# Drexubery/ViewCrafter

Measured on NVIDIA H100. Metric: DDIM denoise-steps/sec @ 576x1024x25f, higher is better.
Workload: dtype f16 (fp32 accumulate; fp32 norms/softmax/update)

## Files before the change

### viewcrafter_b200/csrc/attention.cu

```cuda
#include <cstdlib>

#include "common.cuh"
#include "kernels.h"
#include "wgmma.cuh"

namespace vc {

struct AttnParams {
  CUtensorMap tmap_q, tmap_k, tmap_v;
  __half* out;
  int ldo;
  int Nq, Nk;
  int kv_shared;
  float scale_log2;
  int accumulate;
};

static constexpr int ATT_BM = 128, ATT_D = 64;
static constexpr int ATT_THREADS = 288;
static constexpr int ATT_Q_BYTES = ATT_BM * ATT_D * 2;

template <int BNK>
struct AttnCfg {
  static constexpr int KV_BYTES = BNK * ATT_D * 2;
  static constexpr int SMEM = ATT_Q_BYTES + 4 * KV_BYTES + 1024 + 256;
  static constexpr int MIN_CTAS = BNK == 64 ? 2 : 1;
};

__device__ __forceinline__ float ex2f(float x) {
  float y;
  asm("ex2.approx.ftz.f32 %0, %1;" : "=f"(y) : "f"(x));
  return y;
}

template <int BNK>
__global__ void __launch_bounds__(ATT_THREADS, AttnCfg<BNK>::MIN_CTAS) flash_attn_d64_kernel(const __grid_constant__ AttnParams p) {
  using Cfg = AttnCfg<BNK>;
  extern __shared__ uint8_t smem_raw[];
  uint8_t* smem = reinterpret_cast<uint8_t*>((reinterpret_cast<uintptr_t>(smem_raw) + 1023) & ~uintptr_t(1023));
  uint8_t* sQ = smem;
  uint8_t* sKV = smem + ATT_Q_BYTES;
  uint64_t* bars = reinterpret_cast<uint64_t*>(smem + ATT_Q_BYTES + 4 * Cfg::KV_BYTES);
  uint64_t* q_full = bars + 0;
  uint64_t* kv_full = bars + 1;
  uint64_t* kv_empty = bars + 3;

  const int warp = threadIdx.x >> 5, lane = threadIdx.x & 31;
  const int q0 = blockIdx.x * ATT_BM, head = blockIdx.y, b = blockIdx.z;
  const int bk = p.kv_shared ? 0 : b;
  const int ntiles = (p.Nk + BNK - 1) / BNK;

  if (threadIdx.x == 0) {
    tma_prefetch_desc(&p.tmap_q);
    tma_prefetch_desc(&p.tmap_k);
    tma_prefetch_desc(&p.tmap_v);
    mbar_init(q_full, 1);
    mbar_init(&kv_full[0], 1); mbar_init(&kv_full[1], 1);
    mbar_init(&kv_empty[0], 8); mbar_init(&kv_empty[1], 8);
    fence_barrier_init();
  }
  __syncthreads();

  if (warp == 8) {
    if (elect_one()) {
      mbar_expect_tx(q_full, ATT_Q_BYTES);
      tma_load_4d(sQ, &p.tmap_q, q_full, 0, head, q0, b);
    }
    __syncwarp();
    for (int j = 0; j < ntiles; ++j) {
      const int s = j & 1;
      uint8_t* sk = sKV + s * 2 * Cfg::KV_BYTES;
      if (j >= 2) mbar_wait(&kv_empty[s], ((j >> 1) - 1) & 1);
      if (elect_one()) {
        mbar_expect_tx(&kv_full[s], 2 * Cfg::KV_BYTES);
        tma_load_4d(sk, &p.tmap_k, &kv_full[s], 0, head, j * BNK, bk);
        tma_load_4d(sk + Cfg::KV_BYTES, &p.tmap_v, &kv_full[s], 0, head, j * BNK, bk);
      }
      __syncwarp();
    }
    return;
  }

  const int cw = warp >> 2, wl = warp & 3;
  const uint32_t aQ = smem_u32(sQ) + cw * (64 * ATT_D * 2);
  const float sl2 = p.scale_log2;
  float o[32];
#pragma unroll
  for (int i = 0; i < 32; ++i) o[i] = 0.f;
  float m[2] = {-INFINITY, -INFINITY}, l[2] = {0.f, 0.f};
  mbar_wait(q_full, 0);
  for (int j = 0; j < ntiles; ++j) {
    const int s = j & 1;
    const uint32_t aK = smem_u32(sKV + s * 2 * Cfg::KV_BYTES);
    const uint32_t aV = aK + Cfg::KV_BYTES;
    mbar_wait(&kv_full[s], (j >> 1) & 1);
    float sc[BNK / 2];
    wgmma_fence();
#pragma unroll
    for (int k = 0; k < ATT_D / 16; ++k) Wgmma<BNK>::ss(sc, wgmma_desc_sw128(aQ + 32 * k), wgmma_desc_sw128(aK + 32 * k), k > 0 ? 1 : 0);
    wgmma_commit();
    wgmma_wait<0>();
    wgmma_fence_regs(sc);

    const int valid = p.Nk - j * BNK;
    if (valid < BNK) {
#pragma unroll
      for (int i = 0; i < BNK / 2; ++i) {
        const int col = 8 * (i >> 2) + 2 * (lane & 3) + (i & 1);
        if (col >= valid) sc[i] = -INFINITY;
      }
    }
    float mx[2] = {-INFINITY, -INFINITY};
#pragma unroll
    for (int i = 0; i < BNK / 2; ++i) mx[(i >> 1) & 1] = fmaxf(mx[(i >> 1) & 1], sc[i]);
    float alpha[2], negm[2];
#pragma unroll
    for (int h = 0; h < 2; ++h) {
      mx[h] = fmaxf(mx[h], __shfl_xor_sync(0xffffffffu, mx[h], 1));
      mx[h] = fmaxf(mx[h], __shfl_xor_sync(0xffffffffu, mx[h], 2));
      const float mn = fmaxf(m[h], mx[h] * sl2);
      alpha[h] = ex2f(m[h] - mn);
      m[h] = mn;
      negm[h] = -mn;
      l[h] *= alpha[h];
    }
#pragma unroll
    for (int i = 0; i < 32; ++i) o[i] *= alpha[(i >> 1) & 1];
    uint32_t pa[BNK / 16][4];
#pragma unroll
    for (int kk = 0; kk < BNK / 16; ++kk) {
#pragma unroll
      for (int r = 0; r < 4; ++r) {
        const int i = (2 * kk + (r >> 1)) * 4 + 2 * (r & 1);
        const int h = r & 1;
        const float e0 = ex2f(fmaf(sc[i], sl2, negm[h])), e1 = ex2f(fmaf(sc[i + 1], sl2, negm[h]));
        l[h] += e0 + e1;
        pa[kk][r] = pack_half2(e0, e1);
      }
    }
    wgmma_fence();
#pragma unroll
    for (int kk = 0; kk < BNK / 16; ++kk) Wgmma<64, 1>::rs(o, pa[kk], wgmma_desc_sw128(aV + kk * 16 * 128), 1);
    wgmma_commit();
    wgmma_wait<0>();
    wgmma_fence_regs(o);
    __syncwarp();
    if (lane == 0) mbar_arrive(&kv_empty[s]);
  }

  float inv[2];
#pragma unroll
  for (int h = 0; h < 2; ++h) {
    float t = l[h];
    t += __shfl_xor_sync(0xffffffffu, t, 1);
    t += __shfl_xor_sync(0xffffffffu, t, 2);
    inv[h] = 1.f / t;
  }
#pragma unroll
  for (int h = 0; h < 2; ++h) {
    const int row = q0 + cw * 64 + 16 * wl + (lane >> 2) + 8 * h;
    if (row >= p.Nq) continue;
    __half* op = p.out + ((long long)b * p.Nq + row) * p.ldo + head * ATT_D + 2 * (lane & 3);
#pragma unroll
    for (int jj = 0; jj < 8; ++jj) {
      float v0 = o[jj * 4 + 2 * h] * inv[h], v1 = o[jj * 4 + 2 * h + 1] * inv[h];
      __half2* dst = reinterpret_cast<__half2*>(op + 8 * jj);
      if (p.accumulate) {
        const float2 t = __half22float2(*dst);
        v0 += t.x; v1 += t.y;
      }
      *dst = __floats2half2_rn(v0, v1);
    }
  }
}

static int bn64_mode() {
  static int mode = -2;
  if (mode == -2) { const char* e = getenv("VC_ATTN_BN64"); mode = !e ? -1 : (e[0] == '1' ? 1 : 0); }
  return mode;
}

template <int BNK>
static int launch_attn(const AttnDesc& d, cudaStream_t stream) {
  using Cfg = AttnCfg<BNK>;
  AttnParams p;
  memset(&p, 0, sizeof(p));
  {
    uint64_t dims[4] = {64, (uint64_t)d.heads, (uint64_t)d.Nq, (uint64_t)d.B};
    uint64_t str[3] = {128, (uint64_t)d.ldq * 2, (uint64_t)d.ldq * 2 * d.Nq};
    uint32_t box[4] = {64, 1, ATT_BM, 1};
    int rc = encode_tmap_f16(&p.tmap_q, d.q, 4, dims, str, box);
    if (rc) return rc;
  }
  const int shared = d.kv_batch_stride == 0;
  {
    uint64_t dims[4] = {64, (uint64_t)d.heads, (uint64_t)d.Nk, (uint64_t)(shared ? 1 : d.B)};
    uint64_t strk[3] = {128, (uint64_t)d.ldk * 2, (uint64_t)(shared ? (long long)d.ldk * d.Nk : d.kv_batch_stride) * 2};
    uint64_t strv[3] = {128, (uint64_t)d.ldv * 2, (uint64_t)(shared ? (long long)d.ldv * d.Nk : d.kv_batch_stride) * 2};
    uint32_t box[4] = {64, 1, (uint32_t)BNK, 1};
    int rc = encode_tmap_f16(&p.tmap_k, d.k, 4, dims, strk, box);
    if (rc) return rc;
    rc = encode_tmap_f16(&p.tmap_v, d.v, 4, dims, strv, box);
    if (rc) return rc;
  }
  p.out = d.out; p.ldo = d.ldo; p.Nq = d.Nq; p.Nk = d.Nk; p.kv_shared = shared;
  p.scale_log2 = d.scale * 1.4426950408889634f;
  p.accumulate = d.accumulate;
  static DeviceOnce configured;
  if (device_once_needed(configured)) {
    VC_CHECK_CUDA(cudaFuncSetAttribute(flash_attn_d64_kernel<BNK>, cudaFuncAttributeMaxDynamicSharedMemorySize, Cfg::SMEM));
    device_once_mark(configured);
  }
  dim3 grid((d.Nq + ATT_BM - 1) / ATT_BM, d.heads, d.B);
  flash_attn_d64_kernel<BNK><<<grid, ATT_THREADS, Cfg::SMEM, stream>>>(p);
  VC_CHECK_CUDA(cudaGetLastError());
  return VC_OK;
}

int flash_attn_d64(const AttnDesc& d, cudaStream_t stream) {
  VC_REQUIRE(d.q && d.k && d.v && d.out, "flash_attn: null pointer");
  VC_REQUIRE(d.Nq > 0 && d.Nk > 0 && d.B > 0 && d.heads > 0, "flash_attn: empty problem");
  VC_REQUIRE(d.ldq % 8 == 0 && d.ldk % 8 == 0 && d.ldv % 8 == 0 && d.ldo % 8 == 0, "flash_attn: pitches must be multiples of 8");
  VC_REQUIRE(d.kv_batch_stride % 8 == 0, "flash_attn: kv batch stride must be a multiple of 8");
  const int mode = bn64_mode();
  if (mode == 1 || (mode < 0 && d.Nk <= 1024)) return launch_attn<64>(d, stream);
  return launch_attn<128>(d, stream);
}

}
```

Measured before the change: 2.408.

## Add warp-specialized pipelined flash attention kernel overlapping QK^T and PV wgmma

Adds a new 384-thread attention kernel used for long key sequences (Nk > 1024). It has a producer warpgroup with reduced registers (setmaxnreg), a 4-stage KV TMA ring, and 128-wide KV tiles. The loop issues the next tile's QK^T wgmma together with the current tile's PV wgmma, so softmax overlaps with tensor-core work, and it skips the O rescale when the running max did not change. The aim is to hide softmax and memory latency in the long-sequence attention, at the cost of higher register pressure and one CTA per SM.

```diff
diff --git a/viewcrafter_b200/csrc/attention.cu b/viewcrafter_b200/csrc/attention.cu
--- a/viewcrafter_b200/csrc/attention.cu
+++ b/viewcrafter_b200/csrc/attention.cu
@@ -17,15 +17,19 @@
 };
 
 static constexpr int ATT_BM = 128, ATT_D = 64;
+static constexpr int ATT_Q_BYTES = ATT_BM * ATT_D * 2;
+
 static constexpr int ATT_THREADS = 288;
-static constexpr int ATT_Q_BYTES = ATT_BM * ATT_D * 2;
-
-template <int BNK>
-struct AttnCfg {
-  static constexpr int KV_BYTES = BNK * ATT_D * 2;
-  static constexpr int SMEM = ATT_Q_BYTES + 4 * KV_BYTES + 1024 + 256;
-  static constexpr int MIN_CTAS = BNK == 64 ? 2 : 1;
-};
+static constexpr int ATT_BNK = 64;
+static constexpr int ATT_KV_BYTES = ATT_BNK * ATT_D * 2;
+static constexpr int ATT_SMEM = ATT_Q_BYTES + 4 * ATT_KV_BYTES + 1024 + 256;
+
+static constexpr int ATTP_THREADS = 384;
+static constexpr int ATTP_BNK = 128;
+static constexpr int ATTP_KV_BYTES = ATTP_BNK * ATT_D * 2;
+static constexpr int ATTP_STAGES = 4;
+static constexpr int ATTP_SMEM = ATT_Q_BYTES + ATTP_STAGES * 2 * ATTP_KV_BYTES + 1024 + 256;
+static constexpr int ATTP_PRODUCER_REGS = 24, ATTP_MMA_REGS = 240;
 
 __device__ __forceinline__ float ex2f(float x) {
   float y;
@@ -34,13 +38,89 @@
 }
 
 template <int BNK>
-__global__ void __launch_bounds__(ATT_THREADS, AttnCfg<BNK>::MIN_CTAS) flash_attn_d64_kernel(const __grid_constant__ AttnParams p) {
-  using Cfg = AttnCfg<BNK>;
+__device__ __forceinline__ void softmax_tile(float (&sc)[BNK / 2], float (&m)[2], float (&l)[2], float (&alpha)[2], int valid, float sl2,
+                                             int lane) {
+  if (valid < BNK) {
+#pragma unroll
+    for (int i = 0; i < BNK / 2; ++i) {
+      const int col = 8 * (i >> 2) + 2 * (lane & 3) + (i & 1);
+      if (col >= valid) sc[i] = -INFINITY;
+    }
+  }
+  float mx[2] = {-INFINITY, -INFINITY};
+#pragma unroll
+  for (int i = 0; i < BNK / 2; ++i) mx[(i >> 1) & 1] = fmaxf(mx[(i >> 1) & 1], sc[i]);
+  float negm[2];
+#pragma unroll
+  for (int h = 0; h < 2; ++h) {
+    mx[h] = fmaxf(mx[h], __shfl_xor_sync(0xffffffffu, mx[h], 1));
+    mx[h] = fmaxf(mx[h], __shfl_xor_sync(0xffffffffu, mx[h], 2));
+    const float mn = fmaxf(m[h], mx[h] * sl2);
+    alpha[h] = ex2f(m[h] - mn);
+    m[h] = mn;
+    negm[h] = -mn;
+    l[h] *= alpha[h];
+  }
+#pragma unroll
+  for (int kk = 0; kk < BNK / 16; ++kk) {
+#pragma unroll
+    for (int r = 0; r < 4; ++r) {
+      const int i = (2 * kk + (r >> 1)) * 4 + 2 * (r & 1);
+      const int h = r & 1;
+      const float e0 = ex2f(fmaf(sc[i], sl2, negm[h])), e1 = ex2f(fmaf(sc[i + 1], sl2, negm[h]));
+      l[h] += e0 + e1;
+      sc[i] = e0;
+      sc[i + 1] = e1;
+    }
+  }
+}
+
+template <int BNK>
+__device__ __forceinline__ void pack_p(const float (&e)[BNK / 2], uint32_t (&pa)[BNK / 16][4]) {
+#pragma unroll
+  for (int kk = 0; kk < BNK / 16; ++kk)
+#pragma unroll
+    for (int r = 0; r < 4; ++r) {
+      const int i = (2 * kk + (r >> 1)) * 4 + 2 * (r & 1);
+      pa[kk][r] = pack_half2(e[i], e[i + 1]);
+    }
+}
+
+__device__ __forceinline__ void attn_store(const AttnParams& p, const float (&o)[32], const float (&l)[2], int row0, int b, int head,
+                                           int lane) {
+  float inv[2];
+#pragma unroll
+  for (int h = 0; h < 2; ++h) {
+    float t = l[h];
+    t += __shfl_xor_sync(0xffffffffu, t, 1);
+    t += __shfl_xor_sync(0xffffffffu, t, 2);
+    inv[h] = 1.f / t;
+  }
+#pragma unroll
+  for (int h = 0; h < 2; ++h) {
+    const int row = row0 + (lane >> 2) + 8 * h;
+    if (row >= p.Nq) continue;
+    __half* op = p.out + ((long long)b * p.Nq + row) * p.ldo + head * ATT_D + 2 * (lane & 3);
+#pragma unroll
+    for (int jj = 0; jj < 8; ++jj) {
+      float v0 = o[jj * 4 + 2 * h] * inv[h], v1 = o[jj * 4 + 2 * h + 1] * inv[h];
+      __half2* dst = reinterpret_cast<__half2*>(op + 8 * jj);
+      if (p.accumulate) {
+        const float2 t = __half22float2(*dst);
+        v0 += t.x; v1 += t.y;
+      }
+      *dst = __floats2half2_rn(v0, v1);
+    }
+  }
+}
+
+__global__ void __launch_bounds__(ATT_THREADS, 2) flash_attn_d64_kernel(const __grid_constant__ AttnParams p) {
+  constexpr int BNK = ATT_BNK;
   extern __shared__ uint8_t smem_raw[];
   uint8_t* smem = reinterpret_cast<uint8_t*>((reinterpret_cast<uintptr_t>(smem_raw) + 1023) & ~uintptr_t(1023));
   uint8_t* sQ = smem;
   uint8_t* sKV = smem + ATT_Q_BYTES;
-  uint64_t* bars = reinterpret_cast<uint64_t*>(smem + ATT_Q_BYTES + 4 * Cfg::KV_BYTES);
+  uint64_t* bars = reinterpret_cast<uint64_t*>(smem + ATT_Q_BYTES + 4 * ATT_KV_BYTES);
   uint64_t* q_full = bars + 0;
   uint64_t* kv_full = bars + 1;
   uint64_t* kv_empty = bars + 3;
@@ -69,12 +149,12 @@
     __syncwarp();
     for (int j = 0; j < ntiles; ++j) {
       const int s = j & 1;
-      uint8_t* sk = sKV + s * 2 * Cfg::KV_BYTES;
+      uint8_t* sk = sKV + s * 2 * ATT_KV_BYTES;
       if (j >= 2) mbar_wait(&kv_empty[s], ((j >> 1) - 1) & 1);
       if (elect_one()) {
-        mbar_expect_tx(&kv_full[s], 2 * Cfg::KV_BYTES);
+        mbar_expect_tx(&kv_full[s], 2 * ATT_KV_BYTES);
         tma_load_4d(sk, &p.tmap_k, &kv_full[s], 0, head, j * BNK, bk);
-        tma_load_4d(sk + Cfg::KV_BYTES, &p.tmap_v, &kv_full[s], 0, head, j * BNK, bk);
+        tma_load_4d(sk + ATT_KV_BYTES, &p.tmap_v, &kv_full[s], 0, head, j * BNK, bk);
       }
       __syncwarp();
     }
@@ -91,8 +171,8 @@
   mbar_wait(q_full, 0);
   for (int j = 0; j < ntiles; ++j) {
     const int s = j & 1;
-    const uint32_t aK = smem_u32(sKV + s * 2 * Cfg::KV_BYTES);
-    const uint32_t aV = aK + Cfg::KV_BYTES;
+    const uint32_t aK = smem_u32(sKV + s * 2 * ATT_KV_BYTES);
+    const uint32_t aV = aK + ATT_KV_BYTES;
     mbar_wait(&kv_full[s], (j >> 1) & 1);
     float sc[BNK / 2];
     wgmma_fence();
@@ -102,42 +182,12 @@
     wgmma_wait<0>();
     wgmma_fence_regs(sc);
 
-    const int valid = p.Nk - j * BNK;
-    if (valid < BNK) {
-#pragma unroll
-      for (int i = 0; i < BNK / 2; ++i) {
-        const int col = 8 * (i >> 2) + 2 * (lane & 3) + (i & 1);
-        if (col >= valid) sc[i] = -INFINITY;
-      }
-    }
-    float mx[2] = {-INFINITY, -INFINITY};
-#pragma unroll
-    for (int i = 0; i < BNK / 2; ++i) mx[(i >> 1) & 1] = fmaxf(mx[(i >> 1) & 1], sc[i]);
-    float alpha[2], negm[2];
-#pragma unroll
-    for (int h = 0; h < 2; ++h) {
-      mx[h] = fmaxf(mx[h], __shfl_xor_sync(0xffffffffu, mx[h], 1));
-      mx[h] = fmaxf(mx[h], __shfl_xor_sync(0xffffffffu, mx[h], 2));
-      const float mn = fmaxf(m[h], mx[h] * sl2);
-      alpha[h] = ex2f(m[h] - mn);
-      m[h] = mn;
-      negm[h] = -mn;
-      l[h] *= alpha[h];
-    }
+    float alpha[2];
+    softmax_tile<BNK>(sc, m, l, alpha, p.Nk - j * BNK, sl2, lane);
 #pragma unroll
     for (int i = 0; i < 32; ++i) o[i] *= alpha[(i >> 1) & 1];
     uint32_t pa[BNK / 16][4];
-#pragma unroll
-    for (int kk = 0; kk < BNK / 16; ++kk) {
-#pragma unroll
-      for (int r = 0; r < 4; ++r) {
-        const int i = (2 * kk + (r >> 1)) * 4 + 2 * (r & 1);
-        const int h = r & 1;
-        const float e0 = ex2f(fmaf(sc[i], sl2, negm[h])), e1 = ex2f(fmaf(sc[i + 1], sl2, negm[h]));
-        l[h] += e0 + e1;
-        pa[kk][r] = pack_half2(e0, e1);
-      }
-    }
+    pack_p<BNK>(sc, pa);
     wgmma_fence();
 #pragma unroll
     for (int kk = 0; kk < BNK / 16; ++kk) Wgmma<64, 1>::rs(o, pa[kk], wgmma_desc_sw128(aV + kk * 16 * 128), 1);
@@ -147,31 +197,136 @@
     __syncwarp();
     if (lane == 0) mbar_arrive(&kv_empty[s]);
   }
-
-  float inv[2];
-#pragma unroll
-  for (int h = 0; h < 2; ++h) {
-    float t = l[h];
-    t += __shfl_xor_sync(0xffffffffu, t, 1);
-    t += __shfl_xor_sync(0xffffffffu, t, 2);
-    inv[h] = 1.f / t;
-  }
-#pragma unroll
-  for (int h = 0; h < 2; ++h) {
-    const int row = q0 + cw * 64 + 16 * wl + (lane >> 2) + 8 * h;
-    if (row >= p.Nq) continue;
-    __half* op = p.out + ((long long)b * p.Nq + row) * p.ldo + head * ATT_D + 2 * (lane & 3);
-#pragma unroll
-    for (int jj = 0; jj < 8; ++jj) {
-      float v0 = o[jj * 4 + 2 * h] * inv[h], v1 = o[jj * 4 + 2 * h + 1] * inv[h];
-      __half2* dst = reinterpret_cast<__half2*>(op + 8 * jj);
-      if (p.accumulate) {
-        const float2 t = __half22float2(*dst);
-        v0 += t.x; v1 += t.y;
+  attn_store(p, o, l, q0 + cw * 64 + 16 * wl, b, head, lane);
+}
+
+template <int R, int C>
+__device__ __forceinline__ void wgmma_fence_a(uint32_t (&a)[R][C]) {
+#pragma unroll
+  for (int i = 0; i < R; ++i)
+#pragma unroll
+    for (int c = 0; c < C; ++c) asm volatile("" : "+r"(a[i][c])::"memory");
+}
+
+__global__ void __launch_bounds__(ATTP_THREADS, 1) flash_attn_d64_pipelined_kernel(const __grid_constant__ AttnParams p) {
+  constexpr int BNK = ATTP_BNK;
+  constexpr int STAGES = ATTP_STAGES;
+  extern __shared__ uint8_t smem_raw[];
+  uint8_t* smem = reinterpret_cast<uint8_t*>((reinterpret_cast<uintptr_t>(smem_raw) + 1023) & ~uintptr_t(1023));
+  uint8_t* sQ = smem;
+  uint8_t* sKV = smem + ATT_Q_BYTES;
+  uint64_t* bars = reinterpret_cast<uint64_t*>(smem + ATT_Q_BYTES + STAGES * 2 * ATTP_KV_BYTES);
+  uint64_t* q_full = bars + 0;
+  uint64_t* kv_full = bars + 1;
+  uint64_t* kv_empty = bars + 1 + STAGES;
+
+  const int warp = threadIdx.x >> 5, lane = threadIdx.x & 31;
+  const int q0 = blockIdx.x * ATT_BM, head = blockIdx.y, b = blockIdx.z;
+  const int bk = p.kv_shared ? 0 : b;
+  const int ntiles = (p.Nk + BNK - 1) / BNK;
+
+  if (threadIdx.x == 0) {
+    tma_prefetch_desc(&p.tmap_q);
+    tma_prefetch_desc(&p.tmap_k);
+    tma_prefetch_desc(&p.tmap_v);
+    mbar_init(q_full, 1);
+    for (int s = 0; s < STAGES; ++s) {
+      mbar_init(&kv_full[s], 1);
+      mbar_init(&kv_empty[s], 8);
+    }
+    fence_barrier_init();
+  }
+  __syncthreads();
+
+  if (warp < 4) {
+    setmaxnreg_dec<ATTP_PRODUCER_REGS>();
+    if (warp != 0) return;
+    if (elect_one()) {
+      mbar_expect_tx(q_full, ATT_Q_BYTES);
+      tma_load_4d(sQ, &p.tmap_q, q_full, 0, head, q0, b);
+    }
+    __syncwarp();
+    int s = 0;
+    uint32_t ph = 0;
+    for (int j = 0; j < ntiles; ++j) {
+      mbar_wait(&kv_empty[s], ph ^ 1);
+      if (elect_one()) {
+        uint8_t* sk = sKV + s * 2 * ATTP_KV_BYTES;
+        mbar_expect_tx(&kv_full[s], 2 * ATTP_KV_BYTES);
+        tma_load_4d(sk, &p.tmap_k, &kv_full[s], 0, head, j * BNK, bk);
+        tma_load_4d(sk + ATTP_KV_BYTES, &p.tmap_v, &kv_full[s], 0, head, j * BNK, bk);
       }
-      *dst = __floats2half2_rn(v0, v1);
-    }
-  }
+      __syncwarp();
+      if (++s == STAGES) { s = 0; ph ^= 1; }
+    }
+    return;
+  }
+
+  setmaxnreg_inc<ATTP_MMA_REGS>();
+  const int cw = (warp >> 2) - 1, wl = warp & 3;
+  const float sl2 = p.scale_log2;
+  const uint64_t dQ = wgmma_desc_sw128(smem_u32(sQ) + cw * (64 * ATT_D * 2));
+  const uint64_t dK = wgmma_desc_sw128(smem_u32(sKV));
+  const uint64_t dV = wgmma_desc_sw128(smem_u32(sKV) + ATTP_KV_BYTES);
+  constexpr uint32_t STAGE_DESC = 2 * ATTP_KV_BYTES >> 4;
+  float o[32];
+#pragma unroll
+  for (int i = 0; i < 32; ++i) o[i] = 0.f;
+  float m[2] = {-INFINITY, -INFINITY}, l[2] = {0.f, 0.f};
+  float sc[BNK / 2];
+  uint32_t pa[BNK / 16][4];
+  float alpha[2];
+  mbar_wait(q_full, 0);
+
+  mbar_wait(&kv_full[0], 0);
+  wgmma_fence();
+#pragma unroll
+  for (int k = 0; k < ATT_D / 16; ++k) Wgmma<BNK>::ss(sc, dQ + 2 * k, dK + 2 * k, k > 0 ? 1 : 0);
+  wgmma_commit();
+  wgmma_wait<0>();
+  wgmma_fence_regs(sc);
+  softmax_tile<BNK>(sc, m, l, alpha, p.Nk, sl2, lane);
+  pack_p<BNK>(sc, pa);
+
+  int s = 0;
+  uint32_t ph = 0;
+  for (int j = 1; j < ntiles; ++j) {
+    const int sn = s + 1 == STAGES ? 0 : s + 1;
+    if (sn == 0) ph ^= 1;
+    mbar_wait(&kv_full[sn], ph);
+    wgmma_fence();
+#pragma unroll
+    for (int k = 0; k < ATT_D / 16; ++k) Wgmma<BNK>::ss(sc, dQ + 2 * k, dK + sn * STAGE_DESC + 2 * k, k > 0 ? 1 : 0);
+    wgmma_commit();
+#pragma unroll
+    for (int kk = 0; kk < BNK / 16; ++kk) Wgmma<64, 1>::rs(o, pa[kk], dV + s * STAGE_DESC + kk * (16 * 128 >> 4), 1);
+    wgmma_commit();
+    wgmma_wait<1>();
+    wgmma_fence_regs(sc);
+    softmax_tile<BNK>(sc, m, l, alpha, p.Nk - j * BNK, sl2, lane);
+    wgmma_wait<0>();
+    wgmma_fence_regs(o);
+    wgmma_fence_a(pa);
+    if (!__all_sync(0xffffffffu, alpha[0] == 1.f && alpha[1] == 1.f)) {
+#pragma unroll
+      for (int i = 0; i < 32; ++i) o[i] *= alpha[(i >> 1) & 1];
+    }
+    pack_p<BNK>(sc, pa);
+    __syncwarp();
+    if (lane == 0) mbar_arrive(&kv_empty[s]);
+    s = sn;
+  }
+
+  wgmma_fence();
+#pragma unroll
+  for (int kk = 0; kk < BNK / 16; ++kk) Wgmma<64, 1>::rs(o, pa[kk], dV + s * STAGE_DESC + kk * (16 * 128 >> 4), 1);
+  wgmma_commit();
+  wgmma_wait<0>();
+  wgmma_fence_regs(o);
+  wgmma_fence_a(pa);
+  __syncwarp();
+  if (lane == 0) mbar_arrive(&kv_empty[s]);
+  attn_store(p, o, l, q0 + cw * 64 + 16 * wl, b, head, lane);
 }
 
 static int bn64_mode() {
@@ -180,9 +335,8 @@
   return mode;
 }
 
-template <int BNK>
-static int launch_attn(const AttnDesc& d, cudaStream_t stream) {
-  using Cfg = AttnCfg<BNK>;
+static int launch_attn(const AttnDesc& d, bool pipelined, cudaStream_t stream) {
+  const int bnk = pipelined ? ATTP_BNK : ATT_BNK;
   AttnParams p;
   memset(&p, 0, sizeof(p));
   {
@@ -197,7 +351,7 @@
     uint64_t dims[4] = {64, (uint64_t)d.heads, (uint64_t)d.Nk, (uint64_t)(shared ? 1 : d.B)};
     uint64_t strk[3] = {128, (uint64_t)d.ldk * 2, (uint64_t)(shared ? (long long)d.ldk * d.Nk : d.kv_batch_stride) * 2};
     uint64_t strv[3] = {128, (uint64_t)d.ldv * 2, (uint64_t)(shared ? (long long)d.ldv * d.Nk : d.kv_batch_stride) * 2};
-    uint32_t box[4] = {64, 1, (uint32_t)BNK, 1};
+    uint32_t box[4] = {64, 1, (uint32_t)bnk, 1};
     int rc = encode_tmap_f16(&p.tmap_k, d.k, 4, dims, strk, box);
     if (rc) return rc;
     rc = encode_tmap_f16(&p.tmap_v, d.v, 4, dims, strv, box);
@@ -206,13 +360,22 @@
   p.out = d.out; p.ldo = d.ldo; p.Nq = d.Nq; p.Nk = d.Nk; p.kv_shared = shared;
   p.scale_log2 = d.scale * 1.4426950408889634f;
   p.accumulate = d.accumulate;
-  static DeviceOnce configured;
-  if (device_once_needed(configured)) {
-    VC_CHECK_CUDA(cudaFuncSetAttribute(flash_attn_d64_kernel<BNK>, cudaFuncAttributeMaxDynamicSharedMemorySize, Cfg::SMEM));
-    device_once_mark(configured);
-  }
   dim3 grid((d.Nq + ATT_BM - 1) / ATT_BM, d.heads, d.B);
-  flash_attn_d64_kernel<BNK><<<grid, ATT_THREADS, Cfg::SMEM, stream>>>(p);
+  if (pipelined) {
+    static DeviceOnce configured;
+    if (device_once_needed(configured)) {
+      VC_CHECK_CUDA(cudaFuncSetAttribute(flash_attn_d64_pipelined_kernel, cudaFuncAttributeMaxDynamicSharedMemorySize, ATTP_SMEM));
+      device_once_mark(configured);
+    }
+    flash_attn_d64_pipelined_kernel<<<grid, ATTP_THREADS, ATTP_SMEM, stream>>>(p);
+  } else {
+    static DeviceOnce configured;
+    if (device_once_needed(configured)) {
+      VC_CHECK_CUDA(cudaFuncSetAttribute(flash_attn_d64_kernel, cudaFuncAttributeMaxDynamicSharedMemorySize, ATT_SMEM));
+      device_once_mark(configured);
+    }
+    flash_attn_d64_kernel<<<grid, ATT_THREADS, ATT_SMEM, stream>>>(p);
+  }
   VC_CHECK_CUDA(cudaGetLastError());
   return VC_OK;
 }
@@ -223,8 +386,8 @@
   VC_REQUIRE(d.ldq % 8 == 0 && d.ldk % 8 == 0 && d.ldv % 8 == 0 && d.ldo % 8 == 0, "flash_attn: pitches must be multiples of 8");
   VC_REQUIRE(d.kv_batch_stride % 8 == 0, "flash_attn: kv batch stride must be a multiple of 8");
   const int mode = bn64_mode();
-  if (mode == 1 || (mode < 0 && d.Nk <= 1024)) return launch_attn<64>(d, stream);
-  return launch_attn<128>(d, stream);
-}
-
-}
+  const bool bn64 = mode == 1 || (mode < 0 && d.Nk <= 1024);
+  return launch_attn(d, !bn64, stream);
+}
+
+}
```

Measured after the change: 2.437 (median of 6 runs). 1.2% higher.
